# Shadowfear36/SegHiero

Hardware: AMD Instinct MI355X
Metric: images/sec at 512x512 (ResNet-50 2-level), full train step (higher is better)
Workload: dtype f32 (convolutions: exact 3-way bf16 split of every fp32 operand, 6 bf16 MFMA products, f32 accumulate; rest plain f32)

## Files before the change

seghiero_amd/csrc/conv_bf16x6.hip:

```cpp
#include "conv_x6.h"

template <int MODE, int TM, int TN, int WGM, int WGN, int OCC = 0, int SK = 0, int PROF = 0, int ACT = 0>
__global__ __launch_bounds__(64 * WGM * WGN, OCC ? OCC : ((WGM * WGN) / 4 < 2 ? 2 : (WGM * WGN) / 4)) void conv_x6_kernel(const ConvQ p) {
    constexpr int NT = 64 * WGM * WGN;
    constexpr int BM = 32 * TM * WGM, BN = 32 * TN * WGN, BK = 32;
    constexpr int A_PLANE = BM * ROWB, B_PLANE = BN * ROWB;
    constexpr int RPP = NT / 8;
    constexpr int NA = (BM + RPP - 1) / RPP, NB = (BN + RPP - 1) / RPP;
    static_assert(BM >= RPP && BN >= RPP, "tile too small for the thread count");
    extern __shared__ __attribute__((aligned(16))) unsigned char smem[];

    const int t = threadIdx.x, lane = t & 63, wave = t >> 6;
    const int wm = wave / WGN, wn = wave % WGN, l31 = lane & 31, h = lane >> 5;
    unsigned long long tk0 = 0;
    if constexpr (PROF) tk0 = __builtin_amdgcn_s_memtime();
    const unsigned nblk = (unsigned)p.tiles_m * (unsigned)p.tiles_n;
    const unsigned bid = xcd_remap(blockIdx.x, nblk);
    const int tile_n = bid % p.tiles_n, tile_m = bid / p.tiles_n;
    const int m0 = tile_m * BM, n0 = tile_n * BN;
    int cy = 0, cx = 0, Hc = p.H, Wc = p.W, oy0 = 0, ox0 = 0, nth = p.KH, ntw = p.KW, Mc = p.M, Kt = p.K;
    if constexpr (MODE == DGRAD) {
        if (p.parity) {
            cy = blockIdx.y >> 1; cx = blockIdx.y & 1;
            oy0 = (cy + p.pad) & 1; ox0 = (cx + p.pad) & 1;
// ... 18 lines not shown
    bool b_ok[NB];
    int cur_tap = -1;
#pragma unroll
    for (int i = 0; i < NA; ++i) {
        const int m = m0 + r0 + RPP * i;
        if (m < Mc && (BM % RPP == 0 || r0 + RPP * i < BM)) {
            if constexpr (MODE == FPROP) {
                const int ow = m % p.Wo, q = m / p.Wo, oh = q % p.Ho, n = q / p.Ho;
                a_y[i] = oh * p.stride - p.pad; a_x[i] = ow * p.stride - p.pad; a_nb[i] = n * p.H * p.W;
            } else {
                const int iwc = m % Wc, q = m / Wc, ihc = q % Hc, n = q / Hc;
                const int ih = p.parity ? 2 * ihc + oy0 : ihc, iw = p.parity ? 2 * iwc + ox0 : iwc;
                a_y[i] = ih + p.pad; a_x[i] = iw + p.pad; a_nb[i] = n * p.Ho * p.Wo;
            }
        } else { a_y[i] = -(1 << 28); a_x[i] = 0; a_nb[i] = 0; }
    }
#pragma unroll
    for (int i = 0; i < NB; ++i) {
        const int j = n0 + r0 + RPP * i;
        b_ok[i] = j < p.Nn && (BN % RPP == 0 || r0 + RPP * i < BN);
        b_row[i] = (long long)j * (MODE == FPROP ? p.K : p.Kc);
    }
    long long a_off[NA];
    bool a_ok[NA];
    auto set_tap = [&](int tap) {
        int kh, kw;
        if (MODE == DGRAD && p.parity) { const int ty = tap / ntw; kh = cy + 2 * ty; kw = cx + 2 * (tap - ty * ntw); }
        else { kh = tap / p.KW; kw = tap - kh * p.KW; }
        const int dh = kh * p.dil, dw = kw * p.dil;
#pragma unroll
        for (int i = 0; i < NA; ++i) {
            if constexpr (MODE == FPROP) {
                const int ih = a_y[i] + dh, iw = a_x[i] + dw;
                a_ok[i] = (unsigned)ih < (unsigned)p.H && (unsigned)iw < (unsigned)p.W;
                a_off[i] = (long long)(a_nb[i] + ih * p.W + iw) * p.lda;
            } else {
                int th = a_y[i] - dh, tw = a_x[i] - dw;
                bool ok = th >= 0 && tw >= 0;
                if (p.stride > 1) {
                    ok = ok && (th % p.stride == 0) && (tw % p.stride == 0);
                    th /= p.stride; tw /= p.stride;
                }
                a_ok[i] = ok && th < p.Ho && tw < p.Wo;
                a_off[i] = (long long)(a_nb[i] + th * p.Wo + tw) * p.lda;
            }
        }
    };
    f32x4 ra[NA], rb[NB];
    const f32x4 zero4 = {0.f, 0.f, 0.f, 0.f};

    auto load_tile = [&](int kt) {
        const int kbase = kt * BK;
        int tap, cc;
        if (single_tap) { tap = 0; cc = kbase + 4 * kc; }
        else if (tap_uniform) { tap = kbase / p.Kc; cc = kbase - tap * p.Kc + 4 * kc; }
        else { const int k = kbase + 4 * kc; tap = k / p.Kc; cc = k - tap * p.Kc; }
        const bool kok = (kbase + 4 * kc) < Kt;
        if (!tap_uniform || tap != cur_tap) { set_tap(tap); cur_tap = tap; }
        int wtap = tap;
        if (MODE == DGRAD && p.parity) { const int ty = tap / ntw; wtap = (cy + 2 * ty) * p.KW + cx + 2 * (tap - ty * ntw); }
#pragma unroll
        for (int i = 0; i < NA; ++i) ra[i] = (kok && a_ok[i]) ? ld4(p.a + a_off[i] + cc) : zero4;
#pragma unroll
        for (int i = 0; i < NB; ++i) {
            long long off;
            if constexpr (MODE == FPROP) off = b_row[i] + kbase + 4 * kc;
            else off = (long long)wtap * p.Cin * p.Kc + b_row[i] + cc;
            rb[i] = (kok && b_ok[i]) ? ld4(p.b + off) : zero4;
        }
    };
    const int wr_off = ((((kc >> 1) ^ ((t >> 5) & 3))) << 4) + ((kc & 1) << 3);
    auto store_tile = [&]() {
        unsigned char* As = smem;
        unsigned char* Bs = As + 3 * A_PLANE;
#pragma unroll
        for (int i = 0; i < NA; ++i) {
            if (BM % RPP != 0 && r0 + RPP * i >= BM) continue;
            u32x2 q1, q2, q3;
            split4(ra[i], q1, q2, q3);
            const int off = (r0 + RPP * i) * ROWB + wr_off;
            *reinterpret_cast<u32x2*>(As + off) = q1;
            *reinterpret_cast<u32x2*>(As + A_PLANE + off) = q2;
            *reinterpret_cast<u32x2*>(As + 2 * A_PLANE + off) = q3;
        }
#pragma unroll
        for (int i = 0; i < NB; ++i) {
            if (BN % RPP != 0 && r0 + RPP * i >= BN) continue;
            u32x2 q1, q2, q3;
            split4(rb[i], q1, q2, q3);
            const int off = (r0 + RPP * i) * ROWB + wr_off;
            *reinterpret_cast<u32x2*>(Bs + off) = q1;
            *reinterpret_cast<u32x2*>(Bs + B_PLANE + off) = q2;
            *reinterpret_cast<u32x2*>(Bs + 2 * B_PLANE + off) = q3;
        }
    };

    f32x16 acc[TM][TN];
#pragma unroll
    for (int i = 0; i < TM; ++i)
#pragma unroll
        for (int j = 0; j < TN; ++j)
#pragma unroll
            for (int r = 0; r < 16; ++r) acc[i][j][r] = 0.f;

    const int arow = wm * 32 * TM + l31, brow = wn * 32 * TN + l31;
    const int rd_off[2] = {((h ^ ((l31 >> 2) & 3)) << 4), (((2 + h) ^ ((l31 >> 2) & 3)) << 4)};
    auto compute = [&]() {
        const unsigned char* As = smem;
        const unsigned char* Bs = As + 3 * A_PLANE;
#pragma unroll
        for (int s = 0; s < 2; ++s) {
            bf16x8 bfr[TN][3];
#pragma unroll
            for (int j = 0; j < TN; ++j)
#pragma unroll
                for (int pl = 0; pl < 3; ++pl)
                    bfr[j][pl] = __builtin_bit_cast(bf16x8, *reinterpret_cast<const u32x4*>(Bs + pl * B_PLANE + (brow + 32 * j) * ROWB + rd_off[s]));
#pragma unroll
            for (int i = 0; i < TM; ++i) {
// ... 658 lines not shown
    splitk_reduce_kernel<<<rg, 256, 0, st>>>(p.slab, p.ldslab, p.ksplit, p.M, p.Nn, mode == FPROP ? p.extra : nullptr,
                                             mode == DGRAD ? p.extra : nullptr, p.ldadd, p.c, p.ldc,
                                             (mode == FPROP || p.bnb_y != nullptr) ? p.partials : nullptr, bnb);
    return sh_launch_status();
}
static int splitk_plan(long long M, long long N, long long K, int parity, int scatter, int b16 = 0) {
    if (parity || scatter || (N & 3)) return 1;
    const long long tiles = sh_cdiv(M, 128) * sh_cdiv(N, 128), nkt = sh_cdiv(K, 32);
    static int target6 = 0, minkt6 = 0, target1 = 0, minkt1 = 0;
    if (!target6) {
        const char* e = getenv("SEGHIERO_SK_TARGET"); target6 = e ? atoi(e) : 512; e = getenv("SEGHIERO_SK_MINKT"); minkt6 = e ? atoi(e) : 16;
        e = getenv("SEGHIERO_B16_SK_TARGET"); target1 = e ? atoi(e) : 1; e = getenv("SEGHIERO_B16_SK_MINKT"); minkt1 = e ? atoi(e) : 16;
    }
    const int target = b16 ? target1 : target6, minkt = b16 ? minkt1 : minkt6;
    if (tiles >= (target * 3) / 4 || nkt < 2 * minkt) return 1;
    long long S = sh_cdiv(target, tiles);
    if (S > nkt / minkt) S = nkt / minkt;
    if (S > 8) S = 8;
    return S < 2 ? 1 : (int)S;
}
template <int MODE, int TM, int TN, int WGM, int WGN, int OCC = 0, int SK = 0, int PROF = 0, int ACT = 0>
static int launch_x6(ConvQ& p, hipStream_t st) {
    constexpr int BM = 32 * TM * WGM, BN = 32 * TN * WGN;
    constexpr size_t lds = 3 * (size_t)(BM + BN) * ROWB;
    static bool attr_done = false;
    if (!attr_done) {
        (void)hipFuncSetAttribute(reinterpret_cast<const void*>(&conv_x6_kernel<MODE, TM, TN, WGM, WGN, OCC, SK, PROF, ACT>), hipFuncAttributeMaxDynamicSharedMemorySize, (int)lds);
        attr_done = true;
    }
    p.tiles_m = (int)sh_cdiv(p.M, BM);
    p.tiles_n = (int)sh_cdiv(p.Nn, BN);
    dim3 grid((unsigned)(p.tiles_m * p.tiles_n), p.parity ? 4u : (SK ? (unsigned)p.ksplit : 1u));
    conv_x6_kernel<MODE, TM, TN, WGM, WGN, OCC, SK, PROF, ACT><<<grid, 64 * WGM * WGN, lds, st>>>(p);
    if (SK) return sh_x6_splitk_reduce(p, MODE, st);
    return sh_launch_status();
}
static int x6_variant() { static int v = -1; if (v < 0) { const char* e = getenv("SEGHIERO_X6_VARIANT"); v = e ? atoi(e) : 0; } return v; }
template <int MODE>
static int launch_gemm_x6(ConvQ& p, hipStream_t st) {
    constexpr size_t lds = 2 * 3 * (size_t)(128 + 128) * ROWB_G;
    static bool attr_done = false;
    if (!attr_done) {
        (void)hipFuncSetAttribute(reinterpret_cast<const void*>(&gemm_x6_kernel<MODE>), hipFuncAttributeMaxDynamicSharedMemorySize, (int)lds);
        attr_done = true;
    }
    p.tiles_m = (int)sh_cdiv(p.M, 128);
    p.tiles_n = (int)sh_cdiv(p.Nn, 128);
    gemm_x6_kernel<MODE><<<(unsigned)(p.tiles_m * p.tiles_n), 256, lds, st>>>(p);
    return sh_launch_status();
}
template <int MODE>
static int launch_conv_x6(ConvQ& p, hipStream_t st) {
    const long long M = p.M, N = p.Nn;
    if (p.ksplit > 1) return launch_x6<MODE, 2, 2, 2, 2, 0, 1>(p, st);
    if (x6_variant() != 3 && p.KH * p.KW == 1 && p.stride == 1 && p.pad == 0 && !p.scatter && N >= 96 && p.K >= 1024 &&
        sh_cdiv(M, 128) * sh_cdiv(N, 128) >= 192) {
        p.ldb = (MODE == FPROP) ? p.K : p.Kc;
        return launch_gemm_x6<MODE>(p, st);
    }
    if (N > 128 && sh_cdiv(M, 256) * sh_cdiv(N, 256) >= 512) {
        if (sh_cdiv(N, 192) * 192 * 10 < sh_cdiv(N, 256) * 256 * 9) return launch_x6<MODE, 2, 2, 4, 3>(p, st);
        if (MODE == FPROP && x6_variant() == 7 && p.slab) return launch_x6<FPROP, 2, 2, 4, 4, 0, 0, 1>(p, st);
        return launch_x6<MODE, 2, 2, 4, 4>(p, st);
    }
    if (N > 64 && sh_cdiv(M, 256) * sh_cdiv(N, 128) >= 512) return launch_x6<MODE, 2, 2, 4, 2>(p, st);
    int TN = N <= 64 ? 1 : 2, TM = 2;
    if (sh_cdiv(M, 128) * sh_cdiv(N, 64 * TN) < 512) {
        TM = 1;
        if (TN == 2 && sh_cdiv(M, 64) * sh_cdiv(N, 128) < 512) TN = 1;
    }
    if (M <= 64) TM = 1;
    if (MODE == FPROP && TM == 2 && TN == 2 && x6_variant() == 7 && p.slab) return launch_x6<FPROP, 2, 2, 2, 2, 0, 0, 1>(p, st);
    if (TM == 2 && TN == 2) return launch_x6<MODE, 2, 2, 2, 2>(p, st);
    if (TM == 2 && TN == 1) return launch_x6<MODE, 2, 1, 2, 2>(p, st);
    if (TM == 1 && TN == 2) return launch_x6<MODE, 1, 2, 2, 2>(p, st);
    return launch_x6<MODE, 1, 1, 2, 2>(p, st);
}
static int launch_conv_x6_act(ConvQ& p, hipStream_t st) {
    const long long M = p.M, N = p.Nn;
    if (N > 128 && sh_cdiv(M, 256) * sh_cdiv(N, 256) >= 512) return launch_x6<FPROP, 2, 2, 4, 4, 0, 0, 0, 1>(p, st);
    int TN = N <= 64 ? 1 : 2, TM = 2;
    if (sh_cdiv(M, 128) * sh_cdiv(N, 64 * TN) < 512) {
        TM = 1;
        if (TN == 2 && sh_cdiv(M, 64) * sh_cdiv(N, 128) < 512) TN = 1;
    }
    if (M <= 64) TM = 1;
    if (TM == 2 && TN == 2) return launch_x6<FPROP, 2, 2, 2, 2, 0, 0, 0, 1>(p, st);
    if (TM == 2 && TN == 1) return launch_x6<FPROP, 2, 1, 2, 2, 0, 0, 0, 1>(p, st);
    if (TM == 1 && TN == 2) return launch_x6<FPROP, 1, 2, 2, 2, 0, 0, 0, 1>(p, st);
    return launch_x6<FPROP, 1, 1, 2, 2, 0, 0, 0, 1>(p, st);
}
static bool geom(ConvQ& p, int N, int H, int W, int Cin, int Cout, int KH, int KW, int stride, int pad, int dil) {
    if (N <= 0 || H <= 0 || W <= 0 || Cin <= 0 || Cout <= 0 || KH <= 0 || KW <= 0 || stride <= 0 || dil <= 0 || pad < 0) return false;
    if (Cin % 4 != 0) return false;
    p.N = N; p.H = H; p.W = W; p.Cin = Cin; p.Cout = Cout; p.KH = KH; p.KW = KW; p.stride = stride; p.pad = pad; p.dil = dil;
    p.Ho = (H + 2 * pad - dil * (KH - 1) - 1) / stride + 1;
    p.Wo = (W + 2 * pad - dil * (KW - 1) - 1) / stride + 1;
    if (p.Ho <= 0 || p.Wo <= 0) return false;
    if ((long long)N * H * W >= (1ll << 31) || (long long)N * p.Ho * p.Wo >= (1ll << 31)) return false;
    if ((long long)KH * KW * (long long)(Cin > Cout ? Cin : Cout + 3) >= (1ll << 30)) return false;
    return true;
}

extern "C" int64_t sh_conv_x6_workspace(int which, int N, int H, int W, int Cin, int Cout, int KH, int KW, int stride, int pad, int dil, int mode) {
    ConvQ p{};
    if (!geom(p, N, H, W, Cin, Cout, KH, KW, stride, pad, dil)) return -1;
    long long M, Nn, K;
    int parity = 0;
    if (which == 0) { M = (long long)N * p.Ho * p.Wo; Nn = Cout; K = (long long)KH * KW * Cin; }
    else {
        if (mode != 0) return 0;
        M = (long long)N * H * W; Nn = Cin; K = (long long)KH * KW * ((Cout + 3) & ~3);
        parity = stride == 2 && dil == 1 && KH * KW > 1;
    }
    const int S = splitk_plan(M, Nn, K, parity, 0);
    return S > 1 ? (int64_t)S * M * Nn * 4 : 0;
}
static void use_splitk(ConvQ& p, float* workspace, int64_t workspace_bytes, int b16 = 0) {
    if (x6_variant() == 7 && workspace && workspace_bytes >= (1 << 20)) { p.slab = workspace; return; }
    const int S = splitk_plan(p.M, p.Nn, p.K, p.parity, p.scatter, b16);
    if (S > 1 && workspace && workspace_bytes >= (int64_t)S * p.M * p.Nn * 4) { p.ksplit = S; p.slab = workspace; p.ldslab = p.Nn; }
}
static bool operand_extents(ConvQ& p, int mode) {
    long long a, b;
    if (mode == FPROP) { a = ((long long)p.N * p.H * p.W - 1) * p.lda + p.Cin; b = (long long)p.Cout * p.K; }
    else { a = ((long long)p.N * p.Ho * p.Wo - 1) * p.lda + p.Kc; b = (long long)p.KH * p.KW * p.Cin * p.Kc; }
    if (a * 4 >= (1ll << 31) || b * 4 >= (1ll << 31)) return false;
    p.a_bytes = (unsigned)(a * ((mode == FPROP && (p.act & 1)) ? 2 : 4)); p.b_bytes = (unsigned)(b * 4);
    return true;
}
static int launch_fprop_any(ConvQ& p, hipStream_t st) {
    if (operand_extents(p, FPROP)) { const int rc = sh_x6p_launch(FPROP, p, st); if (rc != SH_X6P_NO) return rc; }
// ... 463 lines not shown
```

seghiero_amd/csrc/conv_x6.h:

```cpp
#pragma once
#include "common.h"
#include <stdlib.h>

enum { FPROP = 0, DGRAD = 1 };

struct ConvQ {
    const float* a;
    const float* b;
    float* c;
    const float* extra;
    float* partials;
    long long lda, ldb, ldc, ldadd;
    int N, H, W, Cin, Ho, Wo, Cout, KH, KW, stride, pad, dil;
    int M, Nn, K, Kc;
    int Kp;
    int Kreal;
    long long bplane;
    int scatter, sH, sW, sstride;
    int parity;
    int kchunk;
    int tiles_m, tiles_n, n_partials;
    const float* act_scale;
    const float* act_shift;
    const float* act_res;
    int act_relu;
    int ksplit;
    float* slab;
    long long ldslab;
    const float* aff_scale;
    const float* aff_shift;
    const float* bnb_y;
    long long bnb_ldy;
    const float* bnb_mean;
    const float* bnb_invstd;
    const float* bnb_scale;
    const float* bnb_shift;
    int bnb_relu;
    const float* bnb_out;
    long long bnb_ldo;
    int ngroups, group_n;
    const float* ga[6]; unsigned ga_bytes[6]; long long glda[6];
    const float* gb[6];
    const float* gsc[6]; const float* gsh[6];
    const float* a2; long long lda2; unsigned a2_bytes;
    const float* lin;
    int act;
    int vec_epi;
    unsigned a_bytes, b_bytes;
};

typedef __bf16 bf16x8 __attribute__((ext_vector_type(8)));
typedef short s16x4 __attribute__((ext_vector_type(4)));
typedef short s16x8 __attribute__((ext_vector_type(8)));
typedef unsigned int u32x2 __attribute__((ext_vector_type(2)));
typedef unsigned int u32x4 __attribute__((ext_vector_type(4)));

__device__ __forceinline__ f32x16 mfma_bf16(bf16x8 a, bf16x8 b, f32x16 c) {
    return __builtin_amdgcn_mfma_f32_32x32x16_bf16(a, b, c, 0, 0, 0);
}

__device__ __forceinline__ void split4(const f32x4 v, u32x2& p1, u32x2& p2, u32x2& p3) {
    unsigned h1[4], h2[4], h3[4];
#pragma unroll
    for (int j = 0; j < 4; ++j) {
        const unsigned u = __float_as_uint(v[j]);
        const float r1 = v[j] - __uint_as_float(u & 0xffff0000u);
        const unsigned u2 = __float_as_uint(r1);
        const float r2 = r1 - __uint_as_float(u2 & 0xffff0000u);
        h1[j] = u; h2[j] = u2; h3[j] = __float_as_uint(r2);
    }
    p1[0] = __builtin_amdgcn_perm(h1[1], h1[0], 0x07060302u); p1[1] = __builtin_amdgcn_perm(h1[3], h1[2], 0x07060302u);
    p2[0] = __builtin_amdgcn_perm(h2[1], h2[0], 0x07060302u); p2[1] = __builtin_amdgcn_perm(h2[3], h2[2], 0x07060302u);
    p3[0] = __builtin_amdgcn_perm(h3[1], h3[0], 0x07060302u); p3[1] = __builtin_amdgcn_perm(h3[3], h3[2], 0x07060302u);
}

#define ROWB 64
#define ROWB_G 80

__device__ __forceinline__ f32x16 mma6(const bf16x8 (&a)[3], const bf16x8 (&b)[3], f32x16 c) {
    c = mfma_bf16(a[2], b[0], c);
    c = mfma_bf16(a[0], b[2], c);
    c = mfma_bf16(a[1], b[1], c);
    c = mfma_bf16(a[1], b[0], c);
    c = mfma_bf16(a[0], b[1], c);
    c = mfma_bf16(a[0], b[0], c);
    return c;
}


__device__ __forceinline__ f32x16 mma3(const bf16x8 a0, const bf16x8 (&b)[3], f32x16 c) {
    c = mfma_bf16(a0, b[2], c);
    c = mfma_bf16(a0, b[1], c);
    c = mfma_bf16(a0, b[0], c);
    return c;
}

__device__ __forceinline__ f32x16 mma3b(const bf16x8 (&a)[3], const bf16x8 b0, f32x16 c) {
    c = mfma_bf16(a[2], b0, c);
    c = mfma_bf16(a[1], b0, c);
    c = mfma_bf16(a[0], b0, c);
    return c;
}
// ... 10 lines not shown
```

seghiero_amd/csrc/conv_x6p.hip:

```cpp
#include "conv_x6.h"

__device__ __forceinline__ int swz_row(int row) { return ((row >> 2) & 3) ^ (row & 2); }

#ifndef SH_W1
#define SH_W1(AFF, EPI) ((AFF) == 2 ? 2 : 3)
#define SH_W2(AFF, EPI) (((AFF) == 2 || (EPI) == 2) ? 3 : 4)
#endif
#ifndef SH_X6P_PART
#define SH_X6P_PART 0
#endif
#define SH_PART(n) (SH_X6P_PART == 0 || SH_X6P_PART == (n))
int sh_x6p_launch_dgrad(ConvQ& p, hipStream_t st, int force);
int sh_x6p_wgrad_l0b0(ConvQ& p, bool aff, int wgm, int wgn, int splits, hipStream_t st);
int sh_x6p_wgrad_l1b0(ConvQ& p, bool aff, int wgm, int wgn, int splits, hipStream_t st);
int sh_x6p_wgrad_l0b1(ConvQ& p, bool aff, int wgm, int wgn, int splits, hipStream_t st);
int sh_x6p_wgrad_l1b1(ConvQ& p, bool aff, int wgm, int wgn, int splits, hipStream_t st);
static int x6p_mode() { static int v = -2; if (v == -2) { const char* e = getenv("SEGHIERO_X6P"); v = e ? atoi(e) : 1; } return v; }
[[maybe_unused]] static int x6p_ws() { static int v = -2; if (v == -2) { const char* e = getenv("SEGHIERO_X6P_WS"); v = e ? atoi(e) : 0; } return v; }
static int x6p_tile() { static int v = -2; if (v == -2) { const char* e = getenv("SEGHIERO_X6P_TILE"); v = e ? atoi(e) : 0; } return v; }
#if SH_PART(1) || SH_PART(2) || defined(SH_X6P_EXP)
template <int MODE, int TM, int TN, int WGM, int WGN, int WPS, int AFF, int EPI, int SK, int TAP, int GRP = 0, int ABF = 0, int WS = 0>
__global__ __launch_bounds__(64 * WGM * WGN * (WS ? 2 : 1), WPS) void conv_x6p_kernel(const ConvQ p) {
    constexpr int NT = 64 * WGM * WGN;
    constexpr int BM = 32 * TM * WGM, BN = 32 * TN * WGN;
    constexpr int A_PLANE = BM * ROWB, B_PLANE = BN * ROWB;
    constexpr int RPP = NT / 4;
    constexpr int NA = BM / RPP, NB = BN / RPP;
    static_assert(BM % RPP == 0 && BN % RPP == 0 && RPP % 64 == 0, "tile / thread-count mismatch");
    extern __shared__ __attribute__((aligned(16))) unsigned char smem[];
    unsigned char* const As = smem;
    unsigned char* const Bs = smem + 3 * A_PLANE;
    float* const coef = reinterpret_cast<float*>(smem + 3 * (A_PLANE + B_PLANE));
    static_assert(AFF != 2 || (MODE == DGRAD && TAP == 0 && !GRP), "the deferred BatchNorm-backward loader exists for 1x1 dgrads");
    static_assert(!ABF || (MODE == FPROP && !GRP) || AFF == 2, "bf16 loader streams: the fprop input, or the y stream of the lin loader");
    constexpr bool A_BF = ABF && MODE == FPROP, A2_BF = ABF && AFF == 2;
    constexpr bool A3 = A_BF && AFF == 0;
    auto load_a4 = [&](const __amdgpu_buffer_rsrc_t& rs, unsigned elem_off, unsigned ok, bool bf) -> f32x4 {
        if (bf) {
            const unsigned voff = ((elem_off * 2u) & ok) | (0x80000000u & ~ok);
            const u32x2 r = __builtin_bit_cast(u32x2, __builtin_amdgcn_raw_buffer_load_b64(rs, voff, 0, 0));
            return f32x4{__uint_as_float(r[0]), __uint_as_float(r[1]), 0.f, 0.f};
        }
        const unsigned voff = ((elem_off * 4u) & ok) | (0x80000000u & ~ok);
        return __builtin_bit_cast(f32x4, __builtin_amdgcn_raw_buffer_load_b128(rs, voff, 0, 0));
    };
    auto widen_a4 = [&](f32x4 v, bool bf) -> f32x4 {
        return bf ? bf16x4_to_f32(sh_u32x2{__float_as_uint(v[0]), __float_as_uint(v[1])}) : v;
    };

    const int t_all = threadIdx.x, t = WS ? (t_all & (NT - 1)) : t_all, lane = t & 63, wave = t >> 6;
    [[maybe_unused]] const bool producer = WS && t_all >= NT;
    static_assert(!WS || (NT & (NT - 1)) == 0, "wave-specialised form: power-of-two wave count");
    const int wm = wave / WGN, wn = wave % WGN, l31 = lane & 31, h = lane >> 5;
    const unsigned nblk = (unsigned)p.tiles_m * (unsigned)p.tiles_n;
    const unsigned bid = xcd_remap(blockIdx.x, nblk);
    const int tile_n = bid % p.tiles_n, tile_m = bid / p.tiles_n;
    const int m0 = tile_m * BM, n0 = tile_n * BN;
    const int grp = GRP ? n0 / p.group_n : 0;
    const float* const a_ptr = GRP ? p.ga[grp] : p.a;
    const float* const b_ptr = GRP ? p.gb[grp] : p.b;
    const unsigned a_bytes = GRP ? p.ga_bytes[grp] : p.a_bytes;
    const int lda = (int)(GRP ? p.glda[grp] : p.lda);
    const float* const sc_ptr = GRP ? p.gsc[grp] : p.aff_scale;
    const float* const sh_ptr = GRP ? p.gsh[grp] : p.aff_shift;
    const float aff_floor = (GRP && sc_ptr == nullptr) ? -INFINITY : 0.f;
    int cy = 0, cx = 0, Hc = p.H, Wc = p.W, oy0 = 0, ox0 = 0, ntw = p.KW, Mc = p.M, Kt = p.K;
    if constexpr (MODE == DGRAD) {
        if (p.parity) {
            cy = blockIdx.y >> 1; cx = blockIdx.y & 1;
            oy0 = (cy + p.pad) & 1; ox0 = (cx + p.pad) & 1;
            Hc = (p.H - oy0 + 1) >> 1; Wc = (p.W - ox0 + 1) >> 1;
            const int nth = (p.KH - cy + 1) >> 1;
            ntw = (p.KW - cx + 1) >> 1;
            Mc = p.N * Hc * Wc; Kt = nth * ntw * p.Kc;
            if (m0 >= Mc) return;
        }
    }
    int q_begin = 0, q_end = (Kt + 15) >> 4;
    if constexpr (SK) {
        const int per = ((q_end + p.ksplit - 1) / p.ksplit + 1) & ~1;
        q_begin = min(q_end, (int)blockIdx.y * per); q_end = min(q_end, q_begin + per);
    }
    const int klim = min(Kt, 16 * q_end);
    const int nq = (q_end - q_begin + 1) & ~1;
    constexpr bool single_tap = TAP == 0, tap_uniform = TAP <= 1;
// ... 18 lines not shown
                const int ow = m % p.Wo, q = m / p.Wo, oh = q % p.Ho, n = q / p.Ho;
                a_y[i] = oh * p.stride - p.pad; a_x[i] = ow * p.stride - p.pad; a_nb[i] = n * p.H * p.W;
            } else {
                const int iwc = m % Wc, q = m / Wc, ihc = q % Hc, n = q / Hc;
                const int ih = p.parity ? 2 * ihc + oy0 : ihc, iw = p.parity ? 2 * iwc + ox0 : iwc;
                a_y[i] = ih + p.pad; a_x[i] = iw + p.pad; a_nb[i] = n * p.Ho * p.Wo;
            }
        } else { a_y[i] = -(1 << 28); a_x[i] = 0; a_nb[i] = 0; }
    }
#pragma unroll
    for (int i = 0; i < NB; ++i) {
        const int j = n0 + r0 + RPP * i;
        b_ok[i] = j < p.Nn ? ~0u : 0u;
        b_row[i] = (GRP ? j - grp * p.group_n : j) * (MODE == FPROP ? p.K : p.Kc);
    }
    int a_off[NA];
    [[maybe_unused]] int a_off2[NA];
    unsigned a_ok[NA];
    auto set_tap = [&](int tap) {
        if (direct) {
#pragma unroll
            for (int i = 0; i < NA; ++i) {
                a_ok[i] = a_y[i] == 0 ? ~0u : 0u;
                a_off[i] = a_nb[i] * lda;
                if constexpr (AFF == 2) a_off2[i] = a_nb[i] * (int)p.lda2;
            }
            return;
        }
        int kh, kw;
        if (MODE == DGRAD && p.parity) { const int ty = tap / ntw; kh = cy + 2 * ty; kw = cx + 2 * (tap - ty * ntw); }
        else { kh = tap / p.KW; kw = tap - kh * p.KW; }
        const int dh = kh * p.dil, dw = kw * p.dil;
#pragma unroll
        for (int i = 0; i < NA; ++i) {
            if constexpr (MODE == FPROP) {
                const int ih = a_y[i] + dh, iw = a_x[i] + dw;
                a_ok[i] = ((unsigned)ih < (unsigned)p.H && (unsigned)iw < (unsigned)p.W) ? ~0u : 0u;
                a_off[i] = (a_nb[i] + ih * p.W + iw) * lda;
            } else {
                int th = a_y[i] - dh, tw = a_x[i] - dw;
                bool ok = th >= 0 && tw >= 0;
                if (p.stride > 1) {
                    ok = ok && (th % p.stride == 0) && (tw % p.stride == 0);
                    th /= p.stride; tw /= p.stride;
                }
                a_ok[i] = (ok && th < p.Ho && tw < p.Wo) ? ~0u : 0u;
                a_off[i] = (a_nb[i] + th * p.Wo + tw) * lda;
                if constexpr (AFF == 2) a_off2[i] = (a_nb[i] + th * p.Wo + tw) * (int)p.lda2;
            }
        }
    };
    auto prepare_tap = [&](int q) {
        if constexpr (TAP == 1) {
            const int tap = (16 * q) / p.Kc;
            if (tap != cur_tap) { set_tap(tap); cur_tap = tap; }
        }
    };
    if constexpr (TAP == 0) { set_tap(0); cur_tap = 0; }
    const f32x4 zero4 = {0.f, 0.f, 0.f, 0.f};
    struct Regs { f32x4 a[NA]; f32x4 a2[AFF == 2 ? NA : 1]; f32x4 b[NB]; int cc; unsigned okm; };
    auto load_half = [&](int q, Regs& R) {
        const int kbase = 16 * q, k = kbase + 4 * kc;
        int tap, cc;
        if constexpr (single_tap) { tap = 0; cc = k; }
        else if constexpr (tap_uniform) { tap = cur_tap; cc = k - tap * p.Kc; }
        else { tap = k / p.Kc; cc = k - tap * p.Kc; set_tap(tap); }
        const unsigned kok = (unsigned)((k - klim) >> 31);
        int wtap = tap;
        if (MODE == DGRAD && p.parity) { const int ty = tap / ntw; wtap = (cy + 2 * ty) * p.KW + cx + 2 * (tap - ty * ntw); }
        R.cc = cc; R.okm = 0;
#pragma unroll
        for (int i = 0; i < NA; ++i) {
            const unsigned ok = kok & a_ok[i];
            R.a[i] = load_a4(rsrc_a, (unsigned)(a_off[i] + cc), ok, A_BF);
            if constexpr (AFF == 2) R.a2[i] = load_a4(rsrc_a2, (unsigned)(a_off2[i] + cc), ok, A2_BF);
            if (AFF) R.okm |= ok & (1u << i);
        }
#pragma unroll
        for (int i = 0; i < NB; ++i) {
            int off;
            if constexpr (MODE == FPROP) off = b_row[i] + k;
            else off = wtap * p.Cin * p.Kc + b_row[i] + cc;
            const unsigned okb = kok & b_ok[i];
            const unsigned voff = (((unsigned)off * 4u) & okb) | (OOB & ~okb);
            R.b[i] = __builtin_bit_cast(f32x4, __builtin_amdgcn_raw_buffer_load_b128(rsrc_b, voff, 0, 0));
        }
    };
    const int swz_w = swz_row(r0);
    auto store_half = [&](Regs& R, int hb) {
        const int off0 = r0 * ROWB + ((((2 * hb) | (kc >> 1)) ^ swz_w) << 4) + ((kc & 1) << 3);
        f32x4 sc = zero4, sh = zero4;
        [[maybe_unused]] f32x4 lmu = zero4, ld_ = zero4;
        if constexpr (AFF) { sc = *reinterpret_cast<const f32x4*>(coef + R.cc); sh = *reinterpret_cast<const f32x4*>(coef + p.Kc + R.cc); }
        if constexpr (AFF == 2) { lmu = *reinterpret_cast<const f32x4*>(coef + 2 * p.Kc + R.cc); ld_ = *reinterpret_cast<const f32x4*>(coef + 3 * p.Kc + R.cc); }
#pragma unroll
        for (int i = 0; i < NA; ++i) {
            if constexpr (A3) {
                *reinterpret_cast<u32x2*>(As + off0 + RPP * i * ROWB) = u32x2{__float_as_uint(R.a[i][0]), __float_as_uint(R.a[i][1])};
                continue;
            }
            f32x4 v = widen_a4(R.a[i], A_BF);
            if constexpr (AFF == 2) {
                const bool ok = (R.okm >> i) & 1u;
                const f32x4 y2 = widen_a4(R.a2[i], A2_BF);
#pragma unroll
                for (int e = 0; e < 4; ++e) { const float w = fmaf(y2[e] - lmu[e], sh[e], fmaf(v[e], sc[e], ld_[e])); v[e] = ok ? w : 0.f; }
            } else if constexpr (AFF) {
                const bool ok = (R.okm >> i) & 1u;
#pragma unroll
                for (int e = 0; e < 4; ++e) { const float w = fmaxf(v[e] * sc[e] + sh[e], aff_floor); v[e] = ok ? w : 0.f; }
            }
            u32x2 q1, q2, q3;
            split4(v, q1, q2, q3);
            const int off = off0 + RPP * i * ROWB;
            *reinterpret_cast<u32x2*>(As + off) = q1;
            *reinterpret_cast<u32x2*>(As + A_PLANE + off) = q2;
            *reinterpret_cast<u32x2*>(As + 2 * A_PLANE + off) = q3;
        }
#pragma unroll
        for (int i = 0; i < NB; ++i) {
            u32x2 q1, q2, q3;
#ifdef SH_ABLATE_BSPLIT
            q1[0] = __float_as_uint(R.b[i][0]); q1[1] = __float_as_uint(R.b[i][1]); q2 = q1; q3[0] = __float_as_uint(R.b[i][2]); q3[1] = __float_as_uint(R.b[i][3]);
#else
            split4(R.b[i], q1, q2, q3);
#endif
            const int off = off0 + RPP * i * ROWB;
            *reinterpret_cast<u32x2*>(Bs + off) = q1;
            *reinterpret_cast<u32x2*>(Bs + B_PLANE + off) = q2;
            *reinterpret_cast<u32x2*>(Bs + 2 * B_PLANE + off) = q3;
        }
    };

    f32x16 acc[TM][TN];
// ... 30 lines not shown
            }
        }
    };

    auto phase_schedule = [&]() {
        constexpr int PA = A3 ? 1 : 3, PP = A3 ? 3 : 6;
        constexpr int NMFMA = TM * TN * PP, NVALU = 30 * ((A3 ? 0 : NA) + NB) + (AFF == 2 ? 16 : 8 * AFF) * NA, NDSW = PA * NA + 3 * NB,
                      NVM = NA + NB + (AFF == 2 ? NA : 0);
        constexpr int VPM = (NVALU + NMFMA - 1) / NMFMA;
        __builtin_amdgcn_sched_group_barrier(0x100, 3 * TN + PA, 0);
#pragma unroll
        for (int g = 0; g < NMFMA; ++g) {
            __builtin_amdgcn_sched_group_barrier(0x008, 1, 0);
            __builtin_amdgcn_sched_group_barrier(0x002, VPM, 0);
            if (g * NDSW / NMFMA != (g + 1) * NDSW / NMFMA) __builtin_amdgcn_sched_group_barrier(0x200, 1, 0);
            if (g * NVM / NMFMA != (g + 1) * NVM / NMFMA) __builtin_amdgcn_sched_group_barrier(0x020, 1, 0);
            if (g % (PP * TN) == 2 && g / (PP * TN) + 1 < TM) __builtin_amdgcn_sched_group_barrier(0x100, PA, 0);
        }
    };
    if constexpr (AFF == 2) {
        for (int c = t_all; c < 4 * p.Kc; c += NT * (WS ? 2 : 1)) coef[c] = p.lin[c];
        __syncthreads();
    } else if constexpr (AFF) {
        for (int c = t_all; c < p.Kc; c += NT * (WS ? 2 : 1)) { coef[c] = sc_ptr ? sc_ptr[c] : 1.f; coef[p.Kc + c] = sh_ptr ? sh_ptr[c] : 0.f; }
        __syncthreads();
    }
    if constexpr (WS) {
        if (producer) {
            Regs R0, R1;
            prepare_tap(q_begin);     load_half(q_begin, R0);
            prepare_tap(q_begin + 1); load_half(q_begin + 1, R1);
            store_half(R0, 0);
            prepare_tap(q_begin + 2); load_half(q_begin + 2, R0);
            __syncthreads();
            for (int j = 0; j < nq; j += 2) {
                prepare_tap(q_begin + j + 3);
                store_half(R1, 1);
                load_half(q_begin + j + 3, R1);
                __syncthreads();
                prepare_tap(q_begin + j + 4);
                store_half(R0, 0);
                load_half(q_begin + j + 4, R0);
                __syncthreads();
            }
            return;
        }
        __syncthreads();
        for (int j = 0; j < nq; j += 2) {
            compute_half(0);
            __syncthreads();
            compute_half(1);
            __syncthreads();
        }
    } else {
    Regs R0, R1;
    prepare_tap(q_begin);     load_half(q_begin, R0);
    prepare_tap(q_begin + 1); load_half(q_begin + 1, R1);
    store_half(R0, 0);
    prepare_tap(q_begin + 2); load_half(q_begin + 2, R0);
    __syncthreads();
    for (int j = 0; j < nq; j += 2) {
        prepare_tap(q_begin + j + 3);
        store_half(R1, 1);
        load_half(q_begin + j + 3, R1);
        compute_half(0);
        phase_schedule();
        __syncthreads();
        prepare_tap(q_begin + j + 4);
        store_half(R0, 0);
        load_half(q_begin + j + 4, R0);
        compute_half(1);
        phase_schedule();
        __syncthreads();
    }
    }

    if constexpr (SK) {
        float* slab = p.slab + (long long)blockIdx.y * p.M * p.ldslab;
#pragma unroll
        for (int j = 0; j < TN; ++j) {
            const int n = n0 + wn * 32 * TN + 32 * j + l31;
#pragma unroll
            for (int i = 0; i < TM; ++i)
#pragma unroll
                for (int r = 0; r < 16; ++r) {
                    const int m = m0 + wm * 32 * TM + 32 * i + (r & 3) + 8 * (r >> 2) + 4 * h;
                    if (m < p.M && n < p.Nn) slab[(long long)m * p.ldslab + n] = acc[i][j][r];
                }
        }
        return;
    }

    static_assert(EPI == 0 || TM % 2 == 0, "statistics epilogues need whole 64-row groups per wave");
    int ncol[TN];
    bool nok[TN];
    float bias[TN];
    [[maybe_unused]] float b_mu[TN], b_is[TN], b_sc[TN], b_sh[TN];
#pragma unroll
    for (int j = 0; j < TN; ++j) {
        ncol[j] = n0 + wn * 32 * TN + 32 * j + l31;
        nok[j] = ncol[j] < p.Nn;
        bias[j] = (MODE == FPROP && p.extra != nullptr && nok[j]) ? p.extra[ncol[j]] : 0.f;
        if constexpr (EPI == 2) {
            b_mu[j] = b_is[j] = b_sc[j] = b_sh[j] = 0.f;
            if (nok[j]) { b_mu[j] = p.bnb_mean[ncol[j]]; b_is[j] = p.bnb_invstd[ncol[j]]; b_sc[j] = p.bnb_scale[ncol[j]]; b_sh[j] = p.bnb_shift[ncol[j]]; }
        }
// ... 135 lines not shown
                if ((i & 1) == 0) { pend_s[j] = s1; pend_q[j] = q1; }
                else {
                    const int pidx = tile_m * (BM / 64) + wm * (TM / 2) + (i >> 1);
                    if (h == 0 && pidx < p.n_partials && nok[j]) {
                        p.partials[((long long)pidx * 2 + 0) * p.Nn + ncol[j]] = pend_s[j] + s1;
                        p.partials[((long long)pidx * 2 + 1) * p.Nn + ncol[j]] = pend_q[j] + q1;
                    }
                }
            }
        }
    }
    }
    if constexpr (MODE == FPROP && EPI == 1) {
        if (p.partials != nullptr) {
            const int wrow0 = m0 + wm * 32 * TM;
#pragma unroll
            for (int pr = 0; pr < TM / 2; ++pr) {
                const int prow0 = wrow0 + 64 * pr;
                const int npr = max(0, min(64, p.M - prow0));
                const int pidx = tile_m * (BM / 64) + wm * (TM / 2) + pr;
#pragma unroll
                for (int j = 0; j < TN; ++j) {
                    float ss = 0.f;
#pragma unroll
                    for (int i = 2 * pr; i < 2 * pr + 2; ++i)
#pragma unroll
                        for (int r = 0; r < 16; ++r) ss += acc[i][j][r];
                    ss += __shfl_xor(ss, 32, 64);
                    const float mean = npr > 0 ? ss / (float)npr : 0.f;
                    float qq = 0.f;
#pragma unroll
                    for (int i = 2 * pr; i < 2 * pr + 2; ++i)
#pragma unroll
                        for (int r = 0; r < 16; ++r) {
                            const int row = wrow0 + 32 * i + (r & 3) + 8 * (r >> 2) + 4 * h;
                            const float dv = acc[i][j][r] - mean;
                            qq += (npr == 64 || row < p.M) ? dv * dv : 0.f;
                        }
                    qq += __shfl_xor(qq, 32, 64);
                    const int n = n0 + wn * 32 * TN + 32 * j + l31;
                    if (h == 0 && pidx < p.n_partials && n < p.Nn) {
                        p.partials[((long long)pidx * 2 + 0) * p.Nn + n] = ss;
                        p.partials[((long long)pidx * 2 + 1) * p.Nn + n] = qq;
                    }
                }
            }
        }
    }
}

template <int MODE, int TM, int TN, int WGM, int WGN, int WPS, int AFF, int EPI, int SK, int TAP, int GRP = 0, int ABF = 0, int WS = 0>
static int launch_x6p(ConvQ& p, hipStream_t st) {
    constexpr int BM = 32 * TM * WGM, BN = 32 * TN * WGN;
    const size_t lds = 3 * (size_t)(BM + BN) * ROWB + (AFF == 2 ? 16 : AFF ? 8 : 0) * (size_t)p.Kc;
    if (lds > 160 * 1024) return SH_X6P_NO;
    static size_t attr_lds = 0;
    if (lds > attr_lds) {
        (void)hipFuncSetAttribute(reinterpret_cast<const void*>(&conv_x6p_kernel<MODE, TM, TN, WGM, WGN, WPS, AFF, EPI, SK, TAP, GRP, ABF, WS>),
                                  hipFuncAttributeMaxDynamicSharedMemorySize, (int)(160 * 1024));
        attr_lds = 160 * 1024;
    }
    p.tiles_m = (int)sh_cdiv(p.M, BM);
    p.tiles_n = (int)sh_cdiv(p.Nn, BN);
    dim3 grid((unsigned)(p.tiles_m * p.tiles_n), p.parity ? 4u : (SK ? (unsigned)p.ksplit : 1u));
    conv_x6p_kernel<MODE, TM, TN, WGM, WGN, WPS, AFF, EPI, SK, TAP, GRP, ABF, WS><<<grid, 64 * WGM * WGN * (WS ? 2 : 1), lds, st>>>(p);
    return sh_launch_status();
}

template <int MODE, int AFF, int EPI, int TAP, int ABF = 0>
static int pick_tile_x6p(ConvQ& p, hipStream_t st, int force) {
    (void)force;
    constexpr int W1 = SH_W1(AFF, EPI), W2 = SH_W2(AFF, EPI);
#ifdef SH_X6P_WS
    if (p.Nn > 64 && x6p_ws()) return launch_x6p<MODE, 2, 2, 2, 2, 2, AFF, EPI, 0, TAP, 0, ABF, 1>(p, st);
#endif
    if (p.Nn > 64) return launch_x6p<MODE, 2, 2, 2, 2, W1, AFF, EPI, 0, TAP, 0, ABF>(p, st);
    return launch_x6p<MODE, 2, 1, 2, 2, W2, AFF, EPI, 0, TAP, 0, ABF>(p, st);
}

template <int MODE, int AFF, int EPI, int ABF = 0>
static int pick_x6p(ConvQ& p, hipStream_t st, int force) {
    if constexpr (AFF == 2) {
        if (p.KH * p.KW != 1) return SH_X6P_NO;
        if (p.ksplit > 1) {
            const int rc = launch_x6p<MODE, 2, 2, 2, 2, 2, 2, 0, 1, 0, 0, ABF>(p, st);
            return rc == SH_OK ? sh_x6_splitk_reduce(p, MODE, st) : rc;
        }
        return pick_tile_x6p<MODE, 2, EPI, 0, ABF>(p, st, force);
    } else {
    if (p.ksplit > 1) {
        int rc;
        if (p.KH * p.KW == 1) rc = launch_x6p<MODE, 2, 2, 2, 2, 3, AFF, 0, 1, 0, 0, ABF>(p, st);
        else if ((p.Kc & 15) == 0) rc = launch_x6p<MODE, 2, 2, 2, 2, 3, AFF, 0, 1, 1, 0, ABF>(p, st);
        else return SH_X6P_NO;
        return rc == SH_OK ? sh_x6_splitk_reduce(p, MODE, st) : rc;
    }
    if (p.KH * p.KW == 1) return pick_tile_x6p<MODE, AFF, EPI, 0, ABF>(p, st, force);
    if ((p.Kc & 15) == 0) return pick_tile_x6p<MODE, AFF, EPI, 1, ABF>(p, st, force);
    if (AFF || EPI == 2 || ABF) return SH_X6P_NO;
    return pick_tile_x6p<MODE, 0, EPI, 2>(p, st, force);
    }
}

#endif
#if SH_PART(1)

int sh_x6p_grouped_launch(ConvQ& p, hipStream_t st) {
    if (p.ngroups < 1 || p.ngroups > 6 || (p.group_n & 127) || p.KH * p.KW != 1) return SH_X6P_NO;
    auto al16 = [](const void* q) { return ((uintptr_t)q & 15) == 0; };
    p.vec_epi = (p.ldc & 3) == 0 && al16(p.c);
    return launch_x6p<FPROP, 2, 2, 2, 2, 3, 1, 1, 0, 0, 1>(p, st);
}

int sh_x6p_launch(int mode, ConvQ& p, hipStream_t st) {
    const bool aff = p.aff_scale != nullptr, bnb = p.bnb_y != nullptr;
    if (!x6p_mode() && !aff && !bnb && !p.lin) return SH_X6P_NO;
    const int force = x6p_tile();
    auto al16 = [](const void* q) { return ((uintptr_t)q & 15) == 0; };
    p.vec_epi = !p.parity && !p.scatter && (p.Nn & 3) == 0 && (p.ldc & 3) == 0 && al16(p.c) &&
                (p.extra == nullptr || (al16(p.extra) && (mode == FPROP || (p.ldadd & 3) == 0))) &&
                (!bnb || ((p.bnb_ldy & 3) == 0 && al16(p.bnb_y) && (p.bnb_out == nullptr || (p.act & 64) || ((p.bnb_ldo & 3) == 0 && al16(p.bnb_out))) && al16(p.bnb_mean) && al16(p.bnb_invstd) && al16(p.bnb_scale) &&
                          al16(p.bnb_shift) && al16(p.partials)));
    if (bnb && !p.vec_epi) return SH_X6P_NO;
    { static int v = -2; if (v == -2) { const char* e = getenv("SEGHIERO_X6P_VEC"); v = e ? atoi(e) : 1; } if (!v && !bnb) p.vec_epi = 0; }
    if ((p.act & 2) && !p.vec_epi) return SH_X6P_NO;
    if (mode == FPROP) {
        if (bnb) return SH_EINVAL;
        if (p.act & 1) return aff ? pick_x6p<FPROP, 1, 1, 1>(p, st, force) : pick_x6p<FPROP, 0, 1, 1>(p, st, force);
        if (aff) return pick_x6p<FPROP, 1, 1>(p, st, force);
        return pick_x6p<FPROP, 0, 1>(p, st, force);
    }
    if (aff) return SH_EINVAL;
    return sh_x6p_launch_dgrad(p, st, force);
}
#endif
#if SH_PART(2)
int sh_x6p_launch_dgrad(ConvQ& p, hipStream_t st, int force) {
    const bool bnb = p.bnb_y != nullptr;
    if (p.lin != nullptr && (p.act & 16)) return bnb ? pick_x6p<DGRAD, 2, 2, 1>(p, st, force) : pick_x6p<DGRAD, 2, 0, 1>(p, st, force);
    if (p.lin != nullptr) return bnb ? pick_x6p<DGRAD, 2, 2>(p, st, force) : pick_x6p<DGRAD, 2, 0>(p, st, force);
    if (bnb) return pick_x6p<DGRAD, 0, 2>(p, st, force);
    return pick_x6p<DGRAD, 0, 0>(p, st, force);
}
#endif

#if SH_X6P_PART == 0 || SH_X6P_PART >= 3
template <int WGM, int WGN, int AFF, int LIN = 0, int XBF = 0>
__global__ __launch_bounds__(64 * WGM * WGN, 2) void conv_wgrad_x6p_kernel(const ConvQ p) {
    constexpr int NT = 64 * WGM * WGN, BM = 64 * WGM, BN = 64 * WGN;
    constexpr bool X3 = XBF && AFF == 0;
    constexpr int AROWB = 2 * BM + 64, BROWB = 2 * BN + 64;
    constexpr int APLANE = 32 * AROWB, BPLANE = 32 * BROWB;
    constexpr int ACPR = BM / 4, BCPR = BN / 4;
    constexpr int AKPP = NT / ACPR, BKPP = NT / BCPR;
    constexpr int NA = 16 / AKPP, NB = 16 / BKPP;
    static_assert(NA >= 1 && NB >= 1, "a loader pass must not straddle the two halves");
    extern __shared__ __attribute__((aligned(16))) unsigned char smem[];
    unsigned char* const As = smem;
    unsigned char* const Bs = smem + 3 * APLANE;
    const int t = threadIdx.x, lane = t & 63, wave = t >> 6;
    const int wm = wave / WGN, wn = wave % WGN, l31 = lane & 31, h = lane >> 5;
    const unsigned nblk = (unsigned)p.tiles_m * (unsigned)p.tiles_n;
    unsigned slice, bid;
    if (p.scatter) { const unsigned kq = blockIdx.x >> 3; slice = (kq / nblk) * 8u + (blockIdx.x & 7u); bid = kq % nblk; }
    else { slice = blockIdx.x / nblk; bid = xcd_remap(blockIdx.x % nblk, nblk); }
    if (slice >= (unsigned)p.ksplit) return;
    const int tile_n = bid % p.tiles_n, tile_m = bid / p.tiles_n;
// ... 242 lines not shown
```

Baseline: 507.4.

## Add row-halo LDS mode reusing staged input rows across all nine 3x3 taps

Adds a TAP==3 path to the pipelined x6 conv kernel for 3x3, stride-1, pad-1, undilated convs whose width is 16, 32 or 64. For each 16-channel chunk it stages a halo of whole input rows in LDS, split into the three bf16 planes, and then reads all nine taps from that halo by shifting offsets. The point is to cut the 9x redundant global loads and bf16 splitting of input data that the plain im2col-style loader does. The K loop is reordered chunk-major (channel chunk outer, tap inner), and the other kernels' loaders are adapted to that ordering too. The cost is more LDS per block, a halo offset table, and a new hand-scheduled pipeline with more index arithmetic and more ways to go wrong.

```diff
diff --git a/seghiero_amd/csrc/conv_bf16x6.hip b/seghiero_amd/csrc/conv_bf16x6.hip
--- a/seghiero_amd/csrc/conv_bf16x6.hip
+++ b/seghiero_amd/csrc/conv_bf16x6.hip
@@ -94,11 +94,16 @@
     auto load_tile = [&](int kt) {
         const int kbase = kt * BK;
         int tap, cc;
-        if (single_tap) { tap = 0; cc = kbase + 4 * kc; }
+        int kphys = kbase + 4 * kc;
+        if (p.chunk_major) {
+            const int q = kphys >> 4, cq = q / 9;
+            tap = q - 9 * cq; cc = 16 * cq + (kphys & 15); kphys = tap * p.Kc + cc;
+        }
+        else if (single_tap) { tap = 0; cc = kbase + 4 * kc; }
         else if (tap_uniform) { tap = kbase / p.Kc; cc = kbase - tap * p.Kc + 4 * kc; }
         else { const int k = kbase + 4 * kc; tap = k / p.Kc; cc = k - tap * p.Kc; }
         const bool kok = (kbase + 4 * kc) < Kt;
-        if (!tap_uniform || tap != cur_tap) { set_tap(tap); cur_tap = tap; }
+        if (p.chunk_major || !tap_uniform || tap != cur_tap) { set_tap(tap); cur_tap = tap; }
         int wtap = tap;
         if (MODE == DGRAD && p.parity) { const int ty = tap / ntw; wtap = (cy + 2 * ty) * p.KW + cx + 2 * (tap - ty * ntw); }
 #pragma unroll
@@ -106,7 +111,7 @@
 #pragma unroll
         for (int i = 0; i < NB; ++i) {
             long long off;
-            if constexpr (MODE == FPROP) off = b_row[i] + kbase + 4 * kc;
+            if constexpr (MODE == FPROP) off = b_row[i] + kphys;
             else off = (long long)wtap * p.Cin * p.Kc + b_row[i] + cc;
             rb[i] = (kok && b_ok[i]) ? ld4(p.b + off) : zero4;
         }
@@ -871,6 +876,7 @@
 template <int MODE>
 static int launch_conv_x6(ConvQ& p, hipStream_t st) {
     const long long M = p.M, N = p.Nn;
+    p.chunk_major = sh_x6_rowhalo_ok(p);
     if (p.ksplit > 1) return launch_x6<MODE, 2, 2, 2, 2, 0, 1>(p, st);
     if (x6_variant() != 3 && p.KH * p.KW == 1 && p.stride == 1 && p.pad == 0 && !p.scatter && N >= 96 && p.K >= 1024 &&
         sh_cdiv(M, 128) * sh_cdiv(N, 128) >= 192) {
@@ -897,6 +903,7 @@
 }
 static int launch_conv_x6_act(ConvQ& p, hipStream_t st) {
     const long long M = p.M, N = p.Nn;
+    p.chunk_major = sh_x6_rowhalo_ok(p);
     if (N > 128 && sh_cdiv(M, 256) * sh_cdiv(N, 256) >= 512) return launch_x6<FPROP, 2, 2, 4, 4, 0, 0, 0, 1>(p, st);
     int TN = N <= 64 ? 1 : 2, TM = 2;
     if (sh_cdiv(M, 128) * sh_cdiv(N, 64 * TN) < 512) {
diff --git a/seghiero_amd/csrc/conv_x6.h b/seghiero_amd/csrc/conv_x6.h
--- a/seghiero_amd/csrc/conv_x6.h
+++ b/seghiero_amd/csrc/conv_x6.h
@@ -47,7 +47,14 @@
     int act;
     int vec_epi;
     unsigned a_bytes, b_bytes;
+    int chunk_major;
 };
+
+static inline bool sh_x6_rowhalo_ok(const ConvQ& p) {
+    if (p.KH != 3 || p.KW != 3 || p.stride != 1 || p.pad != 1 || p.dil != 1 || p.parity || p.scatter) return false;
+    if ((p.Kc & 15) || (p.W != 16 && p.W != 32 && p.W != 64)) return false;
+    return ((long long)p.H * p.W) % 128 == 0 && p.Ho == p.H && p.Wo == p.W;
+}
 
 typedef __bf16 bf16x8 __attribute__((ext_vector_type(8)));
 typedef short s16x4 __attribute__((ext_vector_type(4)));
diff --git a/seghiero_amd/csrc/conv_x6p.hip b/seghiero_amd/csrc/conv_x6p.hip
--- a/seghiero_amd/csrc/conv_x6p.hip
+++ b/seghiero_amd/csrc/conv_x6p.hip
@@ -29,8 +29,11 @@
     static_assert(BM % RPP == 0 && BN % RPP == 0 && RPP % 64 == 0, "tile / thread-count mismatch");
     extern __shared__ __attribute__((aligned(16))) unsigned char smem[];
     unsigned char* const As = smem;
-    unsigned char* const Bs = smem + 3 * A_PLANE;
-    float* const coef = reinterpret_cast<float*>(smem + 3 * (A_PLANE + B_PLANE));
+    const int halo_P = TAP == 3 ? (BM / p.W + 2) * (p.W + 2) : 0;
+    const int a_plane = TAP == 3 ? halo_P * ROWB : A_PLANE;
+    unsigned char* const Bs = smem + 3 * a_plane;
+    [[maybe_unused]] int* const htab = reinterpret_cast<int*>(smem + 3 * (a_plane + B_PLANE));
+    float* const coef = reinterpret_cast<float*>(smem + 3 * (a_plane + B_PLANE) + (TAP == 3 ? ((halo_P * 4 + 15) & ~15) : 0));
     static_assert(AFF != 2 || (MODE == DGRAD && TAP == 0 && !GRP), "the deferred BatchNorm-backward loader exists for 1x1 dgrads");
     static_assert(!ABF || (MODE == FPROP && !GRP) || AFF == 2, "bf16 loader streams: the fprop input, or the y stream of the lin loader");
     constexpr bool A_BF = ABF && MODE == FPROP, A2_BF = ABF && AFF == 2;
@@ -155,7 +158,8 @@
     };
     auto prepare_tap = [&](int q) {
         if constexpr (TAP == 1) {
-            const int tap = (16 * q) / p.Kc;
+            int tap = (16 * q) / p.Kc;
+            if constexpr (ABF) { if (p.chunk_major) tap = q % 9; }
             if (tap != cur_tap) { set_tap(tap); cur_tap = tap; }
         }
     };
@@ -166,7 +170,10 @@
         const int kbase = 16 * q, k = kbase + 4 * kc;
         int tap, cc;
         if constexpr (single_tap) { tap = 0; cc = k; }
-        else if constexpr (tap_uniform) { tap = cur_tap; cc = k - tap * p.Kc; }
+        else if constexpr (tap_uniform) {
+            tap = cur_tap; cc = k - tap * p.Kc;
+            if constexpr (ABF) { if (p.chunk_major) cc = 16 * (q / 9) + 4 * kc; }
+        }
         else { tap = k / p.Kc; cc = k - tap * p.Kc; set_tap(tap); }
         const unsigned kok = (unsigned)((k - klim) >> 31);
         int wtap = tap;
@@ -182,7 +189,7 @@
 #pragma unroll
         for (int i = 0; i < NB; ++i) {
             int off;
-            if constexpr (MODE == FPROP) off = b_row[i] + k;
+            if constexpr (MODE == FPROP) off = b_row[i] + ((ABF && TAP == 1 && p.chunk_major) ? tap * p.Kc + cc : k);
             else off = wtap * p.Cin * p.Kc + b_row[i] + cc;
             const unsigned okb = kok & b_ok[i];
             const unsigned voff = (((unsigned)off * 4u) & okb) | (OOB & ~okb);
@@ -319,6 +326,140 @@
             compute_half(1);
             __syncthreads();
         }
+    } else if constexpr (TAP == 3) {
+    static_assert(BM == 128 && NT == 256 && !GRP && !ABF && !WS && AFF != 2, "row-halo mode: 128-row tiles on four waves, fp32 operands");
+    const int W = p.W, wsh = __ffs(W) - 1, PW = W + 2, HW = p.H * W;
+    const int img = m0 / HW, y0 = (m0 - img * HW) >> wsh;
+    const int nh = (halo_P + 63) >> 6;
+    int c_begin = 0, c_end = p.Kc >> 4;
+    if constexpr (SK) {
+        const int per = (c_end + p.ksplit - 1) / p.ksplit;
+        c_begin = min(c_end, (int)blockIdx.y * per); c_end = min(c_end, c_begin + per);
+    }
+    const int G = 9 * (c_end - c_begin), ng = (G + 1) & ~1;
+    for (int hp = t; hp < halo_P; hp += NT) {
+        const int hy = hp / PW, hx = hp - hy * PW, iy = y0 - 1 + hy, ix = hx - 1;
+        const bool ok = (unsigned)iy < (unsigned)p.H && (unsigned)ix < (unsigned)W;
+        htab[hp] = ok ? (int)((unsigned)((img * p.H + iy) * W + ix) * (unsigned)lda * 4u) : (int)OOB;
+    }
+    __syncthreads();
+    struct HRegs { f32x4 a; f32x4 b[NB]; int cc, slot, half; bool ok; };
+    auto halo_load = [&](int hp, int c, bool live, int& cc, bool& ok) -> f32x4 {
+        const int tv = htab[min(max(hp, 0), halo_P - 1)];
+        ok = live && hp < halo_P && c < c_end && tv >= 0;
+        cc = 16 * min(c, (p.Kc >> 4) - 1) + 4 * kc;
+        const unsigned voff = ok ? (unsigned)tv + (unsigned)cc * 4u : OOB;
+        return __builtin_bit_cast(f32x4, __builtin_amdgcn_raw_buffer_load_b128(rsrc_a, voff, 0, 0));
+    };
+    auto halo_store = [&](f32x4 v, int cc, bool ok, int hp, int half) {
+        if constexpr (AFF) {
+            const f32x4 sc = *reinterpret_cast<const f32x4*>(coef + cc), sh = *reinterpret_cast<const f32x4*>(coef + p.Kc + cc);
+#pragma unroll
+            for (int e = 0; e < 4; ++e) { const float w = fmaxf(v[e] * sc[e] + sh[e], 0.f); v[e] = ok ? w : 0.f; }
+        }
+        u32x2 q1, q2, q3;
+        split4(v, q1, q2, q3);
+        const int off = hp * ROWB + ((((2 * half) | (kc >> 1)) ^ swz_w) << 4) + ((kc & 1) << 3);
+        *reinterpret_cast<u32x2*>(As + off) = q1;
+        *reinterpret_cast<u32x2*>(As + a_plane + off) = q2;
+        *reinterpret_cast<u32x2*>(As + 2 * a_plane + off) = q3;
+    };
+    auto load_phase = [&](int q, HRegs& R) {
+        const int cr = q / 9, tap = q - 9 * cr, cc = 16 * (c_begin + cr) + 4 * kc;
+        const unsigned kok = q < G ? ~0u : 0u;
+#pragma unroll
+        for (int i = 0; i < NB; ++i) {
+            int off;
+            if constexpr (MODE == FPROP) off = b_row[i] + tap * p.Kc + cc;
+            else off = tap * p.Cin * p.Kc + b_row[i] + cc;
+            const unsigned okb = kok & b_ok[i];
+            const unsigned voff = (((unsigned)off * 4u) & okb) | (OOB & ~okb);
+            R.b[i] = __builtin_bit_cast(f32x4, __builtin_amdgcn_raw_buffer_load_b128(rsrc_b, voff, 0, 0));
+        }
+        const int qh = q - 1, crh = qh < 0 ? 0 : qh / 9;
+        R.slot = qh - 9 * crh; R.half = (crh + 1) & 1;
+        R.a = halo_load(r0 + 64 * R.slot, c_begin + crh + 1, qh >= 0, R.cc, R.ok);
+    };
+    auto store_phase = [&](HRegs& R, int hb) {
+        if ((unsigned)R.slot < (unsigned)nh) {
+            const int hp = r0 + 64 * R.slot;
+            if (hp < halo_P) halo_store(R.a, R.cc, R.ok, hp, R.half);
+        }
+        const int off0 = r0 * ROWB + ((((2 * hb) | (kc >> 1)) ^ swz_w) << 4) + ((kc & 1) << 3);
+#pragma unroll
+        for (int i = 0; i < NB; ++i) {
+            u32x2 q1, q2, q3;
+            split4(R.b[i], q1, q2, q3);
+            const int off = off0 + RPP * i * ROWB;
+            *reinterpret_cast<u32x2*>(Bs + off) = q1;
+            *reinterpret_cast<u32x2*>(Bs + B_PLANE + off) = q2;
+            *reinterpret_cast<u32x2*>(Bs + 2 * B_PLANE + off) = q3;
+        }
+    };
+    int hp0[TM];
+#pragma unroll
+    for (int i = 0; i < TM; ++i) { const int mr = arow + 32 * i; hp0[i] = (mr >> wsh) * PW + (mr & (W - 1)); }
+    auto compute_phase = [&](int g, int hb) {
+        const int cr = g / 9, tap = g - 9 * cr, kh = tap / 3, kw = tap - 3 * kh;
+        const int shift = MODE == FPROP ? kh * PW + kw : (2 - kh) * PW + (2 - kw);
+        const int ahalf = cr & 1;
+        const int rd = (((2 * hb) | h) ^ swz_r) << 4;
+        bf16x8 bfr[TN][3];
+#pragma unroll
+        for (int j = 0; j < TN; ++j)
+#pragma unroll
+            for (int pl = 0; pl < 3; ++pl)
+                bfr[j][pl] = __builtin_bit_cast(bf16x8, *reinterpret_cast<const u32x4*>(Bs + pl * B_PLANE + (brow + 32 * j) * ROWB + rd));
+#pragma unroll
+        for (int i = 0; i < TM; ++i) {
+            const int hp = hp0[i] + shift;
+            const int ra = hp * ROWB + ((((2 * ahalf) | h) ^ swz_row(hp)) << 4);
+            bf16x8 af[3];
+#pragma unroll
+            for (int pl = 0; pl < 3; ++pl) af[pl] = __builtin_bit_cast(bf16x8, *reinterpret_cast<const u32x4*>(As + pl * a_plane + ra));
+#pragma unroll
+            for (int j = 0; j < TN; ++j) acc[i][j] = mma6(af, bfr[j], acc[i][j]);
+        }
+    };
+    auto phase_schedule3 = [&]() {
+        constexpr int NMFMA = TM * TN * 6, NVALU = 30 * NB + 16, NDSW = 3 * NB, NVM = NB + 1;
+        constexpr int VPM = (NVALU + NMFMA - 1) / NMFMA;
+        __builtin_amdgcn_sched_group_barrier(0x100, 3 * TN + 3, 0);
+#pragma unroll
+        for (int g = 0; g < NMFMA; ++g) {
+            __builtin_amdgcn_sched_group_barrier(0x008, 1, 0);
+            __builtin_amdgcn_sched_group_barrier(0x002, VPM, 0);
+            if (g * NDSW / NMFMA != (g + 1) * NDSW / NMFMA) __builtin_amdgcn_sched_group_barrier(0x200, 1, 0);
+            if (g * NVM / NMFMA != (g + 1) * NVM / NMFMA) __builtin_amdgcn_sched_group_barrier(0x020, 1, 0);
+            if (g % (6 * TN) == 2 && g / (6 * TN) + 1 < TM) __builtin_amdgcn_sched_group_barrier(0x100, 3, 0);
+        }
+    };
+    {
+        constexpr int NHMAX = 5;
+        f32x4 pre[NHMAX]; int pcc[NHMAX]; bool pok[NHMAX];
+#pragma unroll
+        for (int s2 = 0; s2 < NHMAX; ++s2) pre[s2] = halo_load(r0 + 64 * s2, c_begin, true, pcc[s2], pok[s2]);
+#pragma unroll
+        for (int s2 = 0; s2 < NHMAX; ++s2) if (r0 + 64 * s2 < halo_P) halo_store(pre[s2], pcc[s2], pok[s2], r0 + 64 * s2, 0);
+    }
+    HRegs R0, R1;
+    load_phase(0, R0);
+    load_phase(1, R1);
+    store_phase(R0, 0);
+    load_phase(2, R0);
+    __syncthreads();
+    for (int j = 0; j < ng; j += 2) {
+        store_phase(R1, 1);
+        load_phase(j + 3, R1);
+        compute_phase(j, 0);
+        phase_schedule3();
+        __syncthreads();
+        store_phase(R0, 0);
+        load_phase(j + 4, R0);
+        compute_phase(j + 1, 1);
+        phase_schedule3();
+        __syncthreads();
+    }
     } else {
     Regs R0, R1;
     prepare_tap(q_begin);     load_half(q_begin, R0);
@@ -560,7 +701,8 @@
 template <int MODE, int TM, int TN, int WGM, int WGN, int WPS, int AFF, int EPI, int SK, int TAP, int GRP = 0, int ABF = 0, int WS = 0>
 static int launch_x6p(ConvQ& p, hipStream_t st) {
     constexpr int BM = 32 * TM * WGM, BN = 32 * TN * WGN;
-    const size_t lds = 3 * (size_t)(BM + BN) * ROWB + (AFF == 2 ? 16 : AFF ? 8 : 0) * (size_t)p.Kc;
+    const size_t halo_p = TAP == 3 ? (size_t)(BM / p.W + 2) * (p.W + 2) : 0;
+    const size_t lds = 3 * ((TAP == 3 ? halo_p : (size_t)BM) + BN) * ROWB + ((halo_p * 4 + 15) & ~(size_t)15) + (AFF == 2 ? 16 : AFF ? 8 : 0) * (size_t)p.Kc;
     if (lds > 160 * 1024) return SH_X6P_NO;
     static size_t attr_lds = 0;
     if (lds > attr_lds) {
@@ -596,6 +738,16 @@
         }
         return pick_tile_x6p<MODE, 2, EPI, 0, ABF>(p, st, force);
     } else {
+    if constexpr (!ABF) {
+        if (p.chunk_major) {
+            if (p.ksplit > 1) {
+                const int rc = launch_x6p<MODE, 2, 2, 2, 2, 2, AFF, 0, 1, 3>(p, st);
+                return rc == SH_OK ? sh_x6_splitk_reduce(p, MODE, st) : rc;
+            }
+            if (p.Nn > 64) return launch_x6p<MODE, 2, 2, 2, 2, 2, AFF, EPI, 0, 3>(p, st);
+            return launch_x6p<MODE, 2, 1, 2, 2, 2, AFF, EPI, 0, 3>(p, st);
+        }
+    }
     if (p.ksplit > 1) {
         int rc;
         if (p.KH * p.KW == 1) rc = launch_x6p<MODE, 2, 2, 2, 2, 3, AFF, 0, 1, 0, 0, ABF>(p, st);
@@ -621,6 +773,7 @@
 }
 
 int sh_x6p_launch(int mode, ConvQ& p, hipStream_t st) {
+    p.chunk_major = sh_x6_rowhalo_ok(p);
     const bool aff = p.aff_scale != nullptr, bnb = p.bnb_y != nullptr;
     if (!x6p_mode() && !aff && !bnb && !p.lin) return SH_X6P_NO;
     const int force = x6p_tile();
```

Result: no change. 505.5 (-0.4%).
